# pyannote/pyannote-audio

Hardware: AMD Instinct MI355X
Metric: audio-hours/sec (real-time factor) for speaker-diarization-3.1 pipeline (higher is better)
Workload: dtype f32

## Files before the change

include/pyannote_amd.h:

```cpp
#ifndef PYANNOTE_AMD_H
#define PYANNOTE_AMD_H

#include <stddef.h>
#include <stdint.h>

#ifdef __cplusplus
extern "C" {
#endif

int pa_version(void);
const char* pa_last_error(void);

void pa_prof_enable(int on);
size_t pa_prof_report(char* buf, size_t cap);

#define PA_MAX_LSTM_LAYERS 8
#define PA_MAX_LINEAR 4

typedef struct pa_seg_weights {
  int32_t sinc_stride;
  int32_t lstm_layers;
  int32_t lstm_hidden;
  int32_t lstm_bidir;
  int32_t num_linear;
// ... 31 lines not shown
                 float* mean, float* rstd, void* stream);
int pa_sinc_fir_pool(const float* wav, long wav_len, long chunk_stride, int B, int N, int stride,
                     const float* mean, const float* rstd, float gamma, float beta,
                     const float* filt_packed, float* out, void* stream);
int pa_sinc_fir_span(const float* wav, long wav_len, long span, const float* filt_packed, float* S, void* stream);
int pa_sinc_fix_pool(const float* S, long Pc, int positions_per_chunk_step, int B, int P, const float* mean,
                     const float* rstd, float gamma, float beta, const float* filt_packed, float* tap_sums,
                     float* out, void* stream);
int pa_conv5_pool(const float* xin, int B, int cin, int Lin, const float* in_mean,
                  const float* in_rstd, const float* gam, const float* bet, const float* w_packed,
                  const float* bias64, float* out, void* stream);
int pa_norm_transpose(const float* xin, int B, int T, const float* in_mean, const float* in_rstd,
                      const float* gam, const float* bet, float* X0, void* stream);
int pa_gemm_tn_ex(const float* A, int lda, const float* W, int ldw, const float* bias, const float* Res,
                  float* C, long ldc, int M, int N, int K, int act, int out_mode, void* stream);
int pa_gemm_tn(const float* A, int lda, const float* W, int ldw, const float* bias, float* C, long ldc,
               int M, int N, int K, int act, int out_mode, void* stream);
int pa_gemm_tn_s2(const float* X, int B, int H, int W, int cin, const float* Wt, int ldw, const float* bias, float* C,
                  long ldc, int N, void* stream);
int pa_lstm_rec(const float* xproj, const float* whh_packed, float* out, int ntiles, int ndir, int T,
                void* stream);
int pa_lstm_rec_h(const float* xproj, const float* whh_packed, float* out, int ntiles, int ndir, int T, int H,
                  void* stream);
int pa_classifier(const float* X, int ldx, int K, int ntiles, int T, int B, const float* cw,
                  const float* cb, int NC, const unsigned char* mapping, int S, float* logp,
                  unsigned char* multilabel, void* stream);

#define PA_MAX_RES_BLOCKS 128

typedef struct pa_emb_weights {
  int32_t num_mel;
  int32_t embed_dim;
  int32_t num_layers;
  int32_t num_blocks[4];
  int32_t planes[4];
  int32_t bottleneck;
  const float* fb_window;
  const float* fb_tw256;
  const float* fb_tw512;
  const float* fb_mel_w;
  const int32_t* fb_mel_lo;
  const int32_t* fb_mel_hi;
  const float* stem_w;
  const float* stem_shift;
  const float* blk_w1[PA_MAX_RES_BLOCKS];
  const float* blk_shift1[PA_MAX_RES_BLOCKS];
  const float* blk_w2[PA_MAX_RES_BLOCKS];
  const float* blk_shift2[PA_MAX_RES_BLOCKS];
  const float* blk_u1[PA_MAX_RES_BLOCKS];
  const float* blk_u2[PA_MAX_RES_BLOCKS];
  const float* blk_wsc[PA_MAX_RES_BLOCKS];
  const float* blk_shiftsc[PA_MAX_RES_BLOCKS];
  const float* blk_w3[PA_MAX_RES_BLOCKS];
  const float* blk_shift3[PA_MAX_RES_BLOCKS];
  const float* seg1_w;
  const float* seg1_b;
  const float* blk_v1[PA_MAX_RES_BLOCKS];
  const float* blk_v2[PA_MAX_RES_BLOCKS];
  int32_t fb_center_kernel;
} pa_emb_weights;

int pa_emb_num_fbank_frames(int num_samples);
int pa_emb_num_pool_frames(const pa_emb_weights* w, int num_samples);
size_t pa_emb_workspace_bytes(const pa_emb_weights* w, int num_chunks, int num_samples, int num_masks);
int pa_emb_forward(const pa_emb_weights* w, const float* wav, int64_t wav_len, int64_t chunk_stride,
                   int num_chunks, int num_samples, const float* masks, int num_masks, int mask_frames,
                   const int32_t* nearest_idx, float* emb, void* workspace, size_t workspace_bytes,
                   void* stream);

size_t pa_emb_ragged_workspace_bytes(const pa_emb_weights* w, int num_utterances, int max_samples);
int pa_emb_forward_ragged(const pa_emb_weights* w, const float* wav, int64_t wav_len, const int64_t* offsets,
                          const int32_t* lengths, int num_utterances, int max_samples, const float* masks, float* emb,
                          void* workspace, size_t workspace_bytes, void* stream);

size_t pa_emb_calibrate_workspace_bytes(const pa_emb_weights* w, int num_chunks, int num_samples);
int pa_emb_calibrate_winograd(const pa_emb_weights* w, const float* wav, int64_t wav_len, int64_t chunk_stride,
                              int num_chunks, int num_samples, float* report, float* emb, void* workspace,
                              size_t workspace_bytes, void* stream);
int pa_absmax_diff(const float* got, const float* ref, long n, float* out2, void* stream);

int pa_fbank(const float* wav, long wav_len, long chunk_stride, int B, int N, const float* window,
             const float* tw256, const float* tw512, const float* mel_w, const int* mel_lo,
             const int* mel_hi, int nmel, float* out, int center, void* stream);
int pa_fbank_center_span(const float* fb, int B, int T, int nmel, int kernel, float* out, void* stream);
int pa_resnet_stem(const float* fbank, int B, int T, int F, const float* w9, const float* shift,
                   float* out, void* stream);
int pa_conv3x3(const float* X, int B, int H, int W, int cin, const float* Wg, const float* shift,
               const float* R, float* Y, int cout, int stride, int relu, void* stream);
int pa_winograd_pack_host(const float* conv_weight ,
                          const float* bn_scale , int cout, int cin,
                          float* U_slabs );
int pa_conv3x3_wino(const float* X, int B, int H, int W, int cin, const float* U, const float* shift,
                    const float* R, float* Y, int cout, int relu, void* stream);
int pa_winograd4_pack_host(const float* conv_weight ,
                           const float* bn_scale , int cout, int cin,
                           float* U_slabs );
int pa_conv3x3_wino4(const float* X, int B, int H, int W, int cin, const float* U, const float* shift,
                     const float* R, float* Y, int cout, int relu, void* stream);
int pa_conv3x3_wino4_rows(const float* X, int B, int H, int W, int cin, const float* U, const float* shift,
                          const float* R, float* Y, int cout, int relu, int rows, void* stream);
int pa_conv3x3_wino_rows(const float* X, int B, int H, int W, int cin, const float* U, const float* shift,
                         const float* R, float* Y, int cout, int relu, int y_first, void* stream);
int pa_stats_pool(const float* feat, int B, int Fh, int Tp, int C, const float* masks, int S, int Fm,
                  const int* nearest_idx, float* stats, void* stream);
int pa_fbank_ragged(const float* wav, long wav_len, const int64_t* offsets, const int32_t* lengths, int B,
                    int max_samples, const float* window, const float* tw256, const float* tw512, const float* mel_w,
                    const int* mel_lo, const int* mel_hi, int nmel, float* out, void* stream);
int pa_zero_tail_cols(float* x, int B, int H, int W, int C, const int32_t* lengths, int halvings, void* stream);
int pa_stats_pool_ragged(const float* feat, int B, int Fh, int W, int C, const int32_t* lengths, int halvings,
                         const float* masks, int ld_masks, float* stats, void* stream);

#define PA_W2V_MAX_CONV 8
#define PA_W2V_MAX_LAYERS 24
typedef struct pa_w2v_layer {
  const float* qk_w;
  const float* qk_b;
  const float* v_w;
  const float* out_w;
  const float* out_b;
  const float* ln1_g;
  const float* ln1_b;
  const float* ff1_w;
  const float* ff1_b;
  const float* ff2_w;
  const float* ff2_b;
  const float* ln2_g;
  const float* ln2_b;
  const float* gate_w;
  const float* gate_b;
  const float* gate_const;
} pa_w2v_layer;

typedef struct pa_sser_weights {
  int32_t num_conv;
  int32_t conv_channels[PA_W2V_MAX_CONV];
  int32_t conv_kernel[PA_W2V_MAX_CONV];
  int32_t conv_stride[PA_W2V_MAX_CONV];
  int32_t extractor_layer_norm;
  int32_t embed_dim, num_layers, num_heads, ff_dim, layer_norm_first;
  int32_t pos_kernel, pos_groups;
  int32_t wavlm;
  int32_t use_layer;
  int32_t lstm_layers, lstm_hidden, lstm_bidir, num_linear, linear_hidden, num_classes, num_speakers;
  const float* conv_w[PA_W2V_MAX_CONV];
  const float* conv_b[PA_W2V_MAX_CONV];
  const float* conv_norm_g[PA_W2V_MAX_CONV];
  const float* conv_norm_b[PA_W2V_MAX_CONV];
  const float* proj_ln_g;
  const float* proj_ln_b;
  const float* proj_w;
  const float* proj_b;
  const float* pos_w;
  const float* pos_b;
  const float* enc_ln_g;
  const float* enc_ln_b;
  pa_w2v_layer layers[PA_W2V_MAX_LAYERS];
  float layer_mix[PA_W2V_MAX_LAYERS];
  const float* lstm_wih[PA_MAX_LSTM_LAYERS];
  const float* lstm_bias[PA_MAX_LSTM_LAYERS];
  const float* lstm_whh[PA_MAX_LSTM_LAYERS];
  const float* lin_w[PA_MAX_LINEAR];
  const float* lin_b[PA_MAX_LINEAR];
  const float* cls_w;
  const float* cls_b;
  const uint8_t* powerset_map;
} pa_sser_weights;
// ... 138 lines not shown
```

pyannote-audio_amd/csrc/emb_fbank.hip:

```cpp
#include "common.h"

namespace pa {

constexpr int FB_WIN = 400, FB_SHIFT = 160, FB_NFFT = 512, FB_HALF = 256, FB_NBIN = 257;
constexpr int FB_FPB = 4;

struct cplx {
  float x, y;
};
__device__ __forceinline__ cplx cmul(cplx a, cplx b) {
  return {a.x * b.x - a.y * b.y, a.x * b.y + a.y * b.x};
}

template <bool kRagged>
__global__ __launch_bounds__(256) void k_fbank(const float* __restrict__ wav, long wav_len,
                                               long chunk_stride, int T, float scale, float preemph,
                                               const float* __restrict__ window,
                                               const float2* __restrict__ tw256,
                                               const float2* __restrict__ tw512,
                                               const float* __restrict__ mel_w,
                                               const int* __restrict__ mel_lo,
                                               const int* __restrict__ mel_hi, int nmel, float eps,
                                               float* __restrict__ out, const int64_t* __restrict__ offs,
                                               const int* __restrict__ lens) {
// ... 61 lines not shown
  }
  __syncthreads();

  float2* src = A;
  float2* dst = Bf;
#pragma unroll
  for (int pass = 0; pass < 4; ++pass) {
    const int Ns = 1 << (2 * pass);
    const int j = lane;
    const int k = j & (Ns - 1);
    const int tstep = 64 >> (2 * pass);
    cplx v[4];
#pragma unroll
    for (int r = 0; r < 4; ++r) {
      const float2 d = src[j + 64 * r];
      const float2 w = s_tw256[(r * k * tstep) & 255];
      v[r] = cmul({d.x, d.y}, {w.x, w.y});
    }
    const cplx t0 = {v[0].x + v[2].x, v[0].y + v[2].y};
    const cplx t1 = {v[0].x - v[2].x, v[0].y - v[2].y};
    const cplx t2 = {v[1].x + v[3].x, v[1].y + v[3].y};
    const cplx d13 = {v[1].x - v[3].x, v[1].y - v[3].y};
    const cplx t3 = {d13.y, -d13.x};
    const int j0 = ((j - k) << 2) + k;
    dst[j0] = make_float2(t0.x + t2.x, t0.y + t2.y);
    dst[j0 + Ns] = make_float2(t1.x + t3.x, t1.y + t3.y);
    dst[j0 + 2 * Ns] = make_float2(t0.x - t2.x, t0.y - t2.y);
    dst[j0 + 3 * Ns] = make_float2(t1.x - t3.x, t1.y - t3.y);
    __syncthreads();
    float2* tmp = src;
    src = dst;
    dst = tmp;
  }
#pragma unroll
  for (int i = 0; i < 5; ++i) {
    const int k = lane + 64 * i;
    if (k <= FB_HALF) {
      const float2 zk = src[k & 255];
      const float2 zc0 = src[(FB_HALF - k) & 255];
      const cplx zc = {zc0.x, -zc0.y};
      const cplx e = {0.5f * (zk.x + zc.x), 0.5f * (zk.y + zc.y)};
      const cplx dd = {0.5f * (zk.x - zc.x), 0.5f * (zk.y - zc.y)};
      const cplx o = {dd.y, -dd.x};
      const float2 w = w512[i];
      const cplx wo = cmul(o, {w.x, w.y});
      const float re = e.x + wo.x, im = e.y + wo.y;
      xw[k] = re * re + im * im;
    }
  }
  __syncthreads();
  if (active) {
    for (int m = lane; m < nmel; m += 64) {
      const float* wrow = mel_w + (long)m * FB_NBIN;
      float acc = 0.f;
      const int lo = mel_lo[m], hi = mel_hi[m];
      for (int k0 = lo; k0 <= hi; k0 += 8) {
        float wk[8];
#pragma unroll
        for (int u = 0; u < 8; ++u) wk[u] = k0 + u <= hi ? wrow[k0 + u] : 0.f;
#pragma unroll
        for (int u = 0; u < 8; ++u)
          if (k0 + u <= hi) acc = fmaf(xw[k0 + u], wk[u], acc);
      }
      out[((long)b * T + t) * nmel + m] = logf(fmaxf(acc, eps));
    }
  }
}

__global__ __launch_bounds__(320) void k_fbank_center(float* __restrict__ fb, int T, int nmel) {
  __shared__ float part[4][80];
  const int b = blockIdx.x;
  const int m = threadIdx.x % 80, p = threadIdx.x / 80;
  float* x = fb + (long)b * T * nmel;
  float s = 0.f;
  if (m < nmel)
    for (int t = p; t < T; t += 4) s += x[(long)t * nmel + m];
  part[p][m] = s;
  __syncthreads();
  const float mean = (part[0][m] + part[1][m] + part[2][m] + part[3][m]) / (float)T;
  if (m < nmel)
    for (int t = p; t < T; t += 4) x[(long)t * nmel + m] -= mean;
}

__global__ __launch_bounds__(320) void k_fbank_center_ragged(float* __restrict__ fb, int T, int nmel,
                                                             const int* __restrict__ lens) {
  __shared__ float part[4][80];
  const int b = blockIdx.x;
  const int m = threadIdx.x % 80, p = threadIdx.x / 80;
  const int n = lens[b];
  const int Tb = n < FB_WIN ? 0 : 1 + (n - FB_WIN) / FB_SHIFT;
  float* x = fb + (long)b * T * nmel;
  float s = 0.f;
  if (m < nmel)
    for (int t = p; t < Tb; t += 4) s += x[(long)t * nmel + m];
  part[p][m] = s;
  __syncthreads();
  const float mean = (part[0][m] + part[1][m] + part[2][m] + part[3][m]) / (float)Tb;
  if (m < nmel) {
    for (int t = p; t < Tb; t += 4) x[(long)t * nmel + m] -= mean;
    for (int t = Tb + p; t < T; t += 4) x[(long)t * nmel + m] = 0.f;
  }
}

constexpr int FC_TT = 240, FC_MG = 16, FC_KMAX = 2049;
__global__ __launch_bounds__(256) void k_fbank_center_span(const float* __restrict__ fb, int T, int nmel, int K,
                                                           float* __restrict__ out) {
  extern __shared__ float fc_tile[];
  const int b = blockIdx.z, m0 = blockIdx.y * FC_MG, t0 = blockIdx.x * FC_TT;
  const int half = K >> 1;
  const int m = threadIdx.x & (FC_MG - 1), tl = threadIdx.x >> 4;
  const float* x = fb + (long)b * T * nmel;
  const int rows = FC_TT + K - 1;
  for (int r = tl; r < rows; r += 16) {
    const int t = t0 - half + r;
    fc_tile[r * FC_MG + m] = (t >= 0 && t < T && m0 + m < nmel) ? x[(long)t * nmel + m0 + m] : 0.f;
  }
  __syncthreads();
  if (m0 + m >= nmel) return;
  for (int i = tl; i < FC_TT; i += 16) {
    const int t = t0 + i;
    if (t >= T) break;
    const int lo = t - half < 0 ? 0 : t - half, hi = t + half > T - 1 ? T - 1 : t + half;
    float s = 0.f;
    for (int u = lo; u <= hi; ++u) s += fc_tile[(u - t0 + half) * FC_MG + m];
    out[((long)b * T + t) * nmel + m0 + m] = fc_tile[(i + half) * FC_MG + m] - s / (float)(hi - lo + 1);
  }
}

}

extern "C" {

int pa_fbank_center_span(const float* fb, int B, int T, int nmel, int kernel, float* out, void* stream) {
  PA_REQUIRE(kernel >= 1 && (kernel & 1), "pa_fbank_center_span: the window must be an odd number of frames (got %d)",
             kernel);
  PA_REQUIRE(fb != out, "pa_fbank_center_span: works out of place");
  if (B <= 0 || T <= 0 || nmel <= 0) return 0;
  if (kernel > 2 * T - 1) kernel = 2 * T - 1;
  PA_REQUIRE(kernel <= pa::FC_KMAX,
             "pa_fbank_center_span: a running mean over %d frames of a %d-frame chunk needs more than the LDS holds "
             "(at most %d frames)", kernel, T, pa::FC_KMAX);
  const size_t lds = (size_t)(pa::FC_TT + kernel - 1) * pa::FC_MG * sizeof(float);
  static bool attr_set = false;
  if (!attr_set) {
    (void)hipFuncSetAttribute((const void*)pa::k_fbank_center_span, hipFuncAttributeMaxDynamicSharedMemorySize,
                              (int)((pa::FC_TT + pa::FC_KMAX - 1) * pa::FC_MG * sizeof(float)));
    attr_set = true;
  }
  hipLaunchKernelGGL(pa::k_fbank_center_span, dim3(pa::cdiv(T, pa::FC_TT), pa::cdiv(nmel, pa::FC_MG), B), dim3(256), lds,
                     (hipStream_t)stream, fb, T, nmel, kernel, out);
  PA_CHECK_LAUNCH("pa_fbank_center_span");
  return 0;
}

int pa_fbank(const float* wav, long wav_len, long chunk_stride, int B, int N, const float* window,
             const float* tw256, const float* tw512, const float* mel_w, const int* mel_lo,
             const int* mel_hi, int nmel, float* out, int center, void* stream) {
  PA_REQUIRE(nmel <= 80, "pa_fbank: at most 80 mel bins are built (got %d)", nmel);
  if (B <= 0) return 0;
  PA_REQUIRE(N >= pa::FB_WIN, "pa_fbank: %d samples is shorter than one 25 ms frame", N);
  const int T = 1 + (N - pa::FB_WIN) / pa::FB_SHIFT;
  hipStream_t st = (hipStream_t)stream;
  pa::ProfScope prof("k_fbank", stream, (double)B * T * (5.0 * 512 * 9 + 2.0 * 257 * 3 + 2.0 * 257 * 2),
                     4.0 * B * N + 4.0 * B * T * nmel * (center ? 3 : 1));
  hipLaunchKernelGGL(pa::k_fbank<false>, dim3(pa::cdiv(T, pa::FB_FPB), B), dim3(256), 0, st, wav, wav_len,
                     chunk_stride, T, 32768.0f, 0.97f, window, (const float2*)tw256,
                     (const float2*)tw512, mel_w, mel_lo, mel_hi, nmel, 1.1920928955078125e-07f, out,
                     (const int64_t*)nullptr, (const int*)nullptr);
  PA_CHECK_LAUNCH("pa_fbank");
  if (center) {
    hipLaunchKernelGGL(pa::k_fbank_center, dim3(B), dim3(320), 0, st, out, T, nmel);
    PA_CHECK_LAUNCH("pa_fbank_center");
  }
  return 0;
}

int pa_fbank_ragged(const float* wav, long wav_len, const int64_t* offsets, const int32_t* lengths, int B,
                    int max_samples, const float* window, const float* tw256, const float* tw512, const float* mel_w,
                    const int* mel_lo, const int* mel_hi, int nmel, float* out, void* stream) {
  PA_REQUIRE(nmel <= 80, "pa_fbank_ragged: at most 80 mel bins are built (got %d)", nmel);
  if (B <= 0) return 0;
  PA_REQUIRE(max_samples >= pa::FB_WIN, "pa_fbank_ragged: %d samples is shorter than one 25 ms frame", max_samples);
  const int T = 1 + (max_samples - pa::FB_WIN) / pa::FB_SHIFT;
  hipStream_t st = (hipStream_t)stream;
  pa::ProfScope prof("k_fbank_ragged", stream, (double)B * T * (5.0 * 512 * 9 + 2.0 * 257 * 3 + 2.0 * 257 * 2),
                     4.0 * B * max_samples + 12.0 * B * T * nmel);
  hipLaunchKernelGGL(pa::k_fbank<true>, dim3(pa::cdiv(T, pa::FB_FPB), B), dim3(256), 0, st, wav, wav_len, 0L, T,
                     32768.0f, 0.97f, window, (const float2*)tw256, (const float2*)tw512, mel_w, mel_lo, mel_hi, nmel,
                     1.1920928955078125e-07f, out, offsets, (const int*)lengths);
  PA_CHECK_LAUNCH("pa_fbank_ragged");
  hipLaunchKernelGGL(pa::k_fbank_center_ragged, dim3(B), dim3(320), 0, st, out, T, nmel, (const int*)lengths);
  PA_CHECK_LAUNCH("pa_fbank_center_ragged");
  return 0;
}

}
```

pyannote-audio_amd/csrc/emb_forward.cpp:

```cpp
#include <hip/hip_runtime.h>
#include <stdint.h>
#include <stdlib.h>

#include "../../include/pyannote_amd.h"

namespace pa {
void set_error(const char* fmt, ...);
}

namespace {

struct EmbPlan {
  int B, N, T, F, S;
  int Hs[5], Ws[5];
  size_t fbank, act[4], stats, total, act_elems;
  size_t t2_off, gather_off;
};
inline size_t align64(size_t n) { return (n + 63) & ~(size_t)63; }

inline bool prefer_wino4(int H, int W, int cin) {
  auto up = [](int a, int b) { return (long)((a + b - 1) / b) * b; };
  long p4 = up(H, 4) * up(W, 64);
  const long p4_lin = up(H, 4) * up(W, 4);
  if (p4_lin * 120 <= p4 * 100) p4 = p4_lin * 120 / 100;
// ... 35 lines not shown
  for (int i = 0; i < 3; ++i) p->act[i] = take(p->act_elems);
  p->t2_off = p->gather_off = 0;
  if (w->bottleneck) {
    size_t t1 = 0, t2 = 0, g = 0;
    int cin = w->planes[0];
    for (int l = 0; l < w->num_layers; ++l) {
      const size_t planes = w->planes[l];
      const size_t in_px = (size_t)B * p->Hs[l == 0 ? 1 : l] * p->Ws[l == 0 ? 1 : l];
      const size_t out_px = (size_t)B * p->Hs[l + 1] * p->Ws[l + 1];
      t1 = t1 > in_px * planes ? t1 : in_px * planes;
      t2 = t2 > out_px * planes ? t2 : out_px * planes;
      if (l > 0) g = g > out_px * cin ? g : out_px * cin;
      cin = 4 * (int)planes;
    }
    p->t2_off = align64(t1);
    p->gather_off = p->t2_off + align64(t2);
    p->act[3] = take(p->gather_off + align64(g));
  } else if (calib) {
    p->act[3] = take(p->act_elems);
  }
  const int L = w->num_layers;
  p->stats = take((size_t)B * p->S * 2 * w->planes[L - 1] * ex * p->Hs[L]);
  p->total = o;
  return true;
}

}

extern "C" {

int pa_emb_num_fbank_frames(int num_samples) {
  return num_samples < 400 ? 0 : 1 + (num_samples - 400) / 160;
}

int pa_emb_num_pool_frames(const pa_emb_weights* w, int num_samples) {
  EmbPlan p;
  if (!make_plan(w, 1, num_samples, 1, &p)) return 0;
  return p.Ws[w->num_layers];
}

size_t pa_emb_workspace_bytes(const pa_emb_weights* w, int num_chunks, int num_samples, int num_masks) {
  EmbPlan p;
  if (!make_plan(w, num_chunks, num_samples, num_masks, &p)) return 0;
  return p.total * sizeof(float);
}

}

extern "C" int pa_absmax_diff(const float* got, const float* ref, long n, float* out2, void* stream);


static int emb_forward_impl(const pa_emb_weights* w, const float* wav, int64_t wav_len, int64_t chunk_stride,
                            int num_chunks, int num_samples, const float* masks, int num_masks, int mask_frames,
                            const int32_t* nearest_idx, float* emb, void* workspace, size_t workspace_bytes,
                            void* stream, float* calib, const int64_t* offsets = nullptr,
                            const int32_t* lengths = nullptr) {
  if (num_chunks <= 0) return 0;
  const bool ragged = lengths != nullptr;
  EmbPlan p;
  if (w->num_layers != 4 || !make_plan(w, num_chunks, num_samples, masks ? num_masks : 1, &p, calib != nullptr)) {
    pa::set_error("pa_emb_forward: %d samples is too short (fbank needs >= 400) or bad layer count",
                  num_samples);
    return 3;
  }
  if (workspace_bytes < p.total * sizeof(float)) {
    pa::set_error("pa_emb_forward: workspace too small (%zu < %zu bytes)", workspace_bytes,
                  p.total * sizeof(float));
    return 3;
  }
  float* ws = (float*)workspace;
  const int B = p.B;
  int rc;
#define RUN(call)           \
  do {                      \
    rc = (call);            \
    if (rc != 0) return rc; \
  } while (0)

  const int span = w->fb_center_kernel;
  if (ragged && span != 0) {
    pa::set_error("pa_emb_forward_ragged: fbank_centering_span checkpoints run one launch sequence per length");
    return 3;
  }
  if (ragged)
    RUN(pa_fbank_ragged(wav, wav_len, offsets, lengths, B, p.N, w->fb_window, w->fb_tw256, w->fb_tw512, w->fb_mel_w,
                        w->fb_mel_lo, w->fb_mel_hi, w->num_mel, ws + p.fbank, stream));
  else
    RUN(pa_fbank(wav, wav_len, chunk_stride, B, p.N, w->fb_window, w->fb_tw256, w->fb_tw512, w->fb_mel_w,
                 w->fb_mel_lo, w->fb_mel_hi, w->num_mel, ws + p.fbank, span == 0 ? 1 : 0, stream));
  auto zero_tail = [&](float* X, int l, int C) -> int {
    return ragged ? pa_zero_tail_cols(X, B, p.Hs[l], p.Ws[l], C, lengths, l > 0 ? l - 1 : 0, stream) : 0;
  };
  float* cur = ws + p.act[0];
  float* f1 = ws + p.act[1];
  float* f2 = ws + p.act[2];
  const float* feats = ws + p.fbank;
  if (span != 0) {
    RUN(pa_fbank_center_span(ws + p.fbank, B, p.T, p.F, span, f1, stream));
    feats = f1;
  }
  RUN(pa_resnet_stem(feats, B, p.T, p.F, w->stem_w, w->stem_shift, cur, stream));
  if (!w->bottleneck) RUN(zero_tail(cur, 0, w->planes[0]));

  auto conv_s1 = [&](const float* X, int H, int W, int ci, const float* v, const float* u, const float* wd,
                     const float* shift, const float* R, float* Y, int co, int slot) -> int {
    if (calib != nullptr) {
      float* scratch = ws + p.act[3];
      float* rep = calib + 4 * slot;
      const long n = (long)B * H * W * co;
      int r = pa_conv3x3(X, B, H, W, ci, wd, shift, R, Y, co, 1, 1, stream);
      if (r == 0 && v != nullptr) {
        r = pa_conv3x3_wino4(X, B, H, W, ci, v, shift, R, scratch, co, 1, stream);
        if (r == 0) r = pa_absmax_diff(scratch, Y, n, rep, stream);
      }
      if (r == 0 && u != nullptr) {
        r = pa_conv3x3_wino(X, B, H, W, ci, u, shift, R, scratch, co, 1, stream);
        if (r == 0) r = pa_absmax_diff(scratch, Y, n, rep + 2, stream);
      }
      return r;
    }
    if (v != nullptr && u != nullptr && H % 4 == 2 && H > 4 && split_rows_wanted() && prefer_wino4(H - 2, W, ci)) {
      const int r = pa_conv3x3_wino4_rows(X, B, H, W, ci, v, shift, R, Y, co, 1, H - 2, stream);
      return r != 0 ? r : pa_conv3x3_wino_rows(X, B, H, W, ci, u, shift, R, Y, co, 1, H - 2, stream);
    }
    if (v != nullptr && prefer_wino4(H, W, ci)) return pa_conv3x3_wino4(X, B, H, W, ci, v, shift, R, Y, co, 1, stream);
    if (u != nullptr) return pa_conv3x3_wino(X, B, H, W, ci, u, shift, R, Y, co, 1, stream);
    return pa_conv3x3(X, B, H, W, ci, wd, shift, R, Y, co, 1, 1, stream);
  };

  int blk = 0;
  int cin = w->planes[0];
  if (w->bottleneck) {
    float* nxt = f1;
    float* sc = f2;
    float* tmp = ws + p.act[3];
    for (int l = 0; l < w->num_layers; ++l) {
      const int planes = w->planes[l], cout = 4 * planes;
      for (int i = 0; i < w->num_blocks[l]; ++i, ++blk) {
        if (blk >= PA_MAX_RES_BLOCKS) {
          pa::set_error("pa_emb_forward: more than %d residual blocks", PA_MAX_RES_BLOCKS);
          return 3;
        }
        const int stride = (i == 0 && l > 0) ? 2 : 1;
        const int H = stride == 2 ? p.Hs[l] : p.Hs[l + 1], W = stride == 2 ? p.Ws[l] : p.Ws[l + 1];
        const int Ho = p.Hs[l + 1], Wo = p.Ws[l + 1];
        float* t1 = tmp;
        float* t2 = tmp + p.t2_off;
        RUN(pa_gemm_tn_ex(cur, cin, w->blk_w1[blk], cin, w->blk_shift1[blk], nullptr, t1, planes, B * H * W,
                          planes, cin, 2, 0, stream));
        RUN(zero_tail(t1, stride == 2 ? l : l + 1, planes));
        if (stride == 1 && w->blk_u2[blk] != nullptr)
          RUN(pa_conv3x3_wino(t1, B, H, W, planes, w->blk_u2[blk], w->blk_shift2[blk], nullptr, t2, planes, 1,
                              stream));
        else
          RUN(pa_conv3x3(t1, B, H, W, planes, w->blk_w2[blk], w->blk_shift2[blk], nullptr, t2, planes, stride,
                         1, stream));
        const float* res = cur;
        if (w->blk_wsc[blk] != nullptr) {
          if (stride == 2)
            RUN(pa_gemm_tn_s2(cur, B, H, W, cin, w->blk_wsc[blk], cin, w->blk_shiftsc[blk], sc, cout, cout, stream));
          else
            RUN(pa_gemm_tn_ex(cur, cin, w->blk_wsc[blk], cin, w->blk_shiftsc[blk], nullptr, sc, cout,
                              B * Ho * Wo, cout, cin, 0, 0, stream));
          res = sc;
        } else if (stride != 1 || cin != cout) {
          pa::set_error("pa_emb_forward: block %d needs a shortcut conv but none was given", blk);
          return 3;
        }
        RUN(pa_gemm_tn_ex(t2, planes, w->blk_w3[blk], planes, w->blk_shift3[blk], res, nxt, cout, B * Ho * Wo,
// ... 111 lines not shown
```

pyannote-audio_amd/ffi.py:

```python
from __future__ import annotations

import ctypes as C
from pathlib import Path

import torch

_LIB = None
PA_MAX_LSTM_LAYERS = 8
PA_MAX_LINEAR = 4

c_fp = C.c_void_p


class SegWeights(C.Structure):
    _fields_ = [
        ("sinc_stride", C.c_int32), ("lstm_layers", C.c_int32), ("lstm_hidden", C.c_int32),
        ("lstm_bidir", C.c_int32), ("num_linear", C.c_int32), ("linear_hidden", C.c_int32),
        ("num_classes", C.c_int32), ("num_speakers", C.c_int32),
        ("wav_gamma", C.c_float), ("wav_beta", C.c_float),
        ("sinc_filt", c_fp), ("norm0", c_fp), ("conv1_w", c_fp), ("conv1_b", c_fp), ("norm1", c_fp),
        ("conv2_w", c_fp), ("conv2_b", c_fp), ("norm2", c_fp),
        ("lstm_wih", c_fp * PA_MAX_LSTM_LAYERS), ("lstm_bias", c_fp * PA_MAX_LSTM_LAYERS),
        ("lstm_whh", c_fp * PA_MAX_LSTM_LAYERS),
        ("lin_w", c_fp * PA_MAX_LINEAR), ("lin_b", c_fp * PA_MAX_LINEAR),
# ... 81 lines not shown
    ]


class LibraryNotBuilt(RuntimeError):
    pass


def lib_path() -> Path:
    import os
    if os.environ.get("PA_LIB"):
        return Path(os.environ["PA_LIB"])
    return Path(__file__).resolve().parent / "libpyannote_amd.so"


def load():
    global _LIB
    if _LIB is not None:
        return _LIB
    p = lib_path()
    if not p.exists():
        raise LibraryNotBuilt(
            f"{p} not found: run `python -c 'import __graft_entry__ as g; g.build()'` "
            "(hipcc --offload-arch=gfx950).  There is no CPU fallback.")
    lib = C.CDLL(str(p))
    lib.pa_last_error.restype = C.c_char_p
    lib.pa_version.restype = C.c_int
    lib.pa_seg_workspace_bytes.restype = C.c_size_t
    lib.pa_seg_workspace_bytes.argtypes = [C.POINTER(SegWeights), C.c_int, C.c_int]
    lib.pa_seg_workspace_bytes_strided.restype = C.c_size_t
    lib.pa_seg_workspace_bytes_strided.argtypes = [C.POINTER(SegWeights), C.c_int, C.c_int, C.c_int64]
    lib.pa_seg_num_frames.argtypes = [C.c_int, C.c_int]
    lib.pa_seg_forward.argtypes = [C.POINTER(SegWeights), c_fp, C.c_int64, C.c_int64, C.c_int, C.c_int,
                                   c_fp, c_fp, c_fp, C.c_size_t, c_fp]
    lib.pa_row_stats.argtypes = [c_fp, C.c_long, C.c_long, C.c_int, C.c_int, C.c_float, c_fp, c_fp, c_fp]
    lib.pa_sinc_fir_pool.argtypes = [c_fp, C.c_long, C.c_long, C.c_int, C.c_int, C.c_int, c_fp, c_fp,
                                     C.c_float, C.c_float, c_fp, c_fp, c_fp]
    lib.pa_sinc_fir_span.argtypes = [c_fp, C.c_long, C.c_long, c_fp, c_fp, c_fp]
    lib.pa_sinc_fix_pool.argtypes = [c_fp, C.c_long, C.c_int, C.c_int, C.c_int, c_fp, c_fp, C.c_float, C.c_float,
                                     c_fp, c_fp, c_fp, c_fp]
    lib.pa_conv5_pool.argtypes = [c_fp, C.c_int, C.c_int, C.c_int, c_fp, c_fp, c_fp, c_fp, c_fp, c_fp,
                                  c_fp, c_fp]
    lib.pa_norm_transpose.argtypes = [c_fp, C.c_int, C.c_int, c_fp, c_fp, c_fp, c_fp, c_fp, c_fp]
    lib.pa_gemm_tn_ex.argtypes = [c_fp, C.c_int, c_fp, C.c_int, c_fp, c_fp, c_fp, C.c_long, C.c_int, C.c_int,
                                  C.c_int, C.c_int, C.c_int, c_fp]
    lib.pa_gemm_tn.argtypes = [c_fp, C.c_int, c_fp, C.c_int, c_fp, c_fp, C.c_long, C.c_int, C.c_int,
                               C.c_int, C.c_int, C.c_int, c_fp]
    lib.pa_lstm_rec.argtypes = [c_fp, c_fp, c_fp, C.c_int, C.c_int, C.c_int, c_fp]
    lib.pa_classifier.argtypes = [c_fp, C.c_int, C.c_int, C.c_int, C.c_int, C.c_int, c_fp, c_fp,
                                  C.c_int, c_fp, C.c_int, c_fp, c_fp, c_fp]
    lib.pa_prof_enable.argtypes = [C.c_int]
    lib.pa_prof_enable.restype = None
    lib.pa_prof_report.argtypes = [C.c_char_p, C.c_size_t]
    lib.pa_prof_report.restype = C.c_size_t
    _declare_optional(lib)
    _LIB = lib
    return lib


_OPTIONAL: list[tuple] = [
    ("pa_emb_num_fbank_frames", [C.c_int], C.c_int),
    ("pa_emb_num_pool_frames", [C.POINTER(EmbWeights), C.c_int], C.c_int),
    ("pa_emb_workspace_bytes", [C.POINTER(EmbWeights), C.c_int, C.c_int, C.c_int], C.c_size_t),
    ("pa_emb_forward", [C.POINTER(EmbWeights), c_fp, C.c_int64, C.c_int64, C.c_int, C.c_int, c_fp,
                        C.c_int, C.c_int, c_fp, c_fp, c_fp, C.c_size_t, c_fp], C.c_int),
    ("pa_emb_ragged_workspace_bytes", [C.POINTER(EmbWeights), C.c_int, C.c_int], C.c_size_t),
    ("pa_emb_forward_ragged", [C.POINTER(EmbWeights), c_fp, C.c_int64, c_fp, c_fp, C.c_int, C.c_int, c_fp, c_fp,
                               c_fp, C.c_size_t, c_fp], C.c_int),
    ("pa_fbank_ragged", [c_fp, C.c_long, c_fp, c_fp, C.c_int, C.c_int, c_fp, c_fp, c_fp, c_fp, c_fp, c_fp, C.c_int,
                         c_fp, c_fp], C.c_int),
    ("pa_zero_tail_cols", [c_fp, C.c_int, C.c_int, C.c_int, C.c_int, c_fp, C.c_int, c_fp], C.c_int),
    ("pa_stats_pool_ragged", [c_fp, C.c_int, C.c_int, C.c_int, C.c_int, c_fp, C.c_int, c_fp, C.c_int, c_fp, c_fp],
     C.c_int),
    ("pa_emb_calibrate_workspace_bytes", [C.POINTER(EmbWeights), C.c_int, C.c_int], C.c_size_t),
    ("pa_emb_calibrate_winograd", [C.POINTER(EmbWeights), c_fp, C.c_int64, C.c_int64, C.c_int, C.c_int, c_fp, c_fp,
                                   c_fp, C.c_size_t, c_fp], C.c_int),
    ("pa_lstm_rec_h", [c_fp, c_fp, c_fp, C.c_int, C.c_int, C.c_int, C.c_int, c_fp], C.c_int),
    ("pa_absmax_diff", [c_fp, c_fp, C.c_long, c_fp, c_fp], C.c_int),
    ("pa_gemm_tn_s2", [c_fp, C.c_int, C.c_int, C.c_int, C.c_int, c_fp, C.c_int, c_fp, c_fp, C.c_long, C.c_int,
                       c_fp], C.c_int),
    ("pa_gemm_tn_batched", [c_fp, C.c_int, C.c_long, C.c_long, c_fp, C.c_int, C.c_long, C.c_long, c_fp, c_fp, C.c_long,
                            C.c_long, C.c_long, C.c_int, C.c_int, C.c_int, C.c_int, C.c_int, C.c_int, c_fp], C.c_int),
    ("pa_fbank", [c_fp, C.c_long, C.c_long, C.c_int, C.c_int, c_fp, c_fp, c_fp, c_fp, c_fp, c_fp,
                  C.c_int, c_fp, C.c_int, c_fp], C.c_int),
    ("pa_fbank_center_span", [c_fp, C.c_int, C.c_int, C.c_int, C.c_int, c_fp, c_fp], C.c_int),
    ("pa_resnet_stem", [c_fp, C.c_int, C.c_int, C.c_int, c_fp, c_fp, c_fp, c_fp], C.c_int),
    ("pa_conv3x3", [c_fp, C.c_int, C.c_int, C.c_int, C.c_int, c_fp, c_fp, c_fp, c_fp, C.c_int, C.c_int,
                    C.c_int, c_fp], C.c_int),
    ("pa_conv3x3_wino", [c_fp, C.c_int, C.c_int, C.c_int, C.c_int, c_fp, c_fp, c_fp, c_fp, C.c_int, C.c_int,
                         c_fp], C.c_int),
    ("pa_conv3x3_wino4", [c_fp, C.c_int, C.c_int, C.c_int, C.c_int, c_fp, c_fp, c_fp, c_fp, C.c_int, C.c_int,
                          c_fp], C.c_int),
    ("pa_conv3x3_wino4_rows", [c_fp, C.c_int, C.c_int, C.c_int, C.c_int, c_fp, c_fp, c_fp, c_fp, C.c_int, C.c_int,
                               C.c_int, c_fp], C.c_int),
    ("pa_conv3x3_wino_rows", [c_fp, C.c_int, C.c_int, C.c_int, C.c_int, c_fp, c_fp, c_fp, c_fp, C.c_int, C.c_int,
                              C.c_int, c_fp], C.c_int),
    ("pa_pdist_f64", [c_fp, C.c_int, C.c_int, c_fp, c_fp], C.c_int),
    ("pa_cdist_cosine_f64", [c_fp, C.c_int, c_fp, C.c_int, C.c_int, c_fp, c_fp, c_fp], C.c_int),
    ("pa_centroid_means", [c_fp, C.c_int, c_fp, c_fp, C.c_int, c_fp, c_fp], C.c_int),
    ("pa_linkage_workspace_bytes", [C.c_int], C.c_size_t),
    ("pa_linkage_centroid_f64", [c_fp, C.c_int, c_fp, c_fp, C.c_size_t, c_fp], C.c_int),
    ("pa_linkage_centroid_f64_ex", [c_fp, C.c_int, c_fp, c_fp, C.c_size_t, C.c_int, c_fp], C.c_int),
    ("pa_seg_chunk_stats", [c_fp, C.c_int, C.c_int, C.c_int, c_fp, c_fp, c_fp], C.c_int),
    ("pa_embedding_masks", [c_fp, C.c_int, C.c_int, C.c_int, c_fp, C.c_int, C.c_int, c_fp, c_fp], C.c_int),
    ("pa_speaker_count", [c_fp, C.c_int, C.c_int, C.c_int, c_fp, C.c_int, c_fp, c_fp, c_fp], C.c_int),
    ("pa_cluster_activations", [c_fp, C.c_int, C.c_int, C.c_int, c_fp, c_fp, C.c_int, C.c_int, c_fp, c_fp],
     C.c_int),
    ("pa_topk_binarize", [c_fp, c_fp, C.c_int, C.c_int, C.c_int, c_fp, c_fp, c_fp], C.c_int),
    ("pa_topk_binarize_f32", [c_fp, c_fp, C.c_int, C.c_int, C.c_int, c_fp, c_fp, c_fp], C.c_int),
    ("pa_binarize_hysteresis", [c_fp, C.c_int, C.c_int, C.c_int, C.c_float, C.c_float, C.c_int, c_fp, c_fp],
     C.c_int),
    ("pa_cluster_max", [c_fp, C.c_int, C.c_int, C.c_int, c_fp, C.c_int, c_fp, c_fp], C.c_int),
    ("pa_aggregate", [c_fp, C.c_int, C.c_int, C.c_int, c_fp, C.c_int, c_fp, c_fp, C.c_float, C.c_float, C.c_int,
                      c_fp, c_fp], C.c_int),
    ("pa_binarize_regions_workspace_bytes", [C.c_int, C.c_int, C.c_int], C.c_size_t),
    ("pa_binarize_regions", [c_fp, C.c_int, C.c_int, c_fp, c_fp, c_fp, c_fp, C.c_double, C.c_double, C.c_double,
                             C.c_int, c_fp, c_fp, c_fp, c_fp, C.c_size_t, c_fp], C.c_int),
    ("pa_resample_poly", [c_fp, C.c_long, c_fp, C.c_int, C.c_int, C.c_int, C.c_int, c_fp, C.c_long, c_fp],
     C.c_int),
    ("pa_plda_transform", [c_fp, C.c_int, C.c_int, C.c_int, C.c_int, c_fp, c_fp, c_fp, c_fp, c_fp, c_fp, c_fp],
     C.c_int),
    ("pa_vbx_workspace_bytes", [C.c_int, C.c_int, C.c_int], C.c_size_t),
    ("pa_vbx_iteration", [c_fp, c_fp, C.c_int, C.c_int, C.c_int, C.c_double, C.c_double, C.c_int, c_fp, c_fp,
                          c_fp, C.c_size_t, c_fp], C.c_int),
    ("pa_stats_pool", [c_fp, C.c_int, C.c_int, C.c_int, C.c_int, c_fp, C.c_int, C.c_int, c_fp, c_fp,
                       c_fp], C.c_int),
    ("pa_stats_pool_rows", [c_fp, C.c_int, C.c_int, C.c_int, C.c_int, C.c_int, c_fp, C.c_int, C.c_int, c_fp,
                            c_fp, C.c_int, c_fp, c_fp, c_fp], C.c_int),
    ("pa_sser_num_frames", [C.POINTER(SserWeights), C.c_int], C.c_int),
    ("pa_sser_workspace_bytes", [C.POINTER(SserWeights), C.c_int, C.c_int], C.c_size_t),
    ("pa_sser_forward", [C.POINTER(SserWeights), c_fp, C.c_int64, C.c_int64, C.c_int, C.c_int, c_fp, c_fp, c_fp,
                         c_fp, C.c_size_t, c_fp], C.c_int),
    ("pa_xvec_num_frames", [C.POINTER(XvecWeights), C.c_int], C.c_int),
    ("pa_xvec_workspace_bytes", [C.POINTER(XvecWeights), C.c_int, C.c_int, C.c_int], C.c_size_t),
    ("pa_xvec_forward", [C.POINTER(XvecWeights), c_fp, C.c_int64, C.c_int64, C.c_int, C.c_int, c_fp,
                         C.c_int, C.c_int, c_fp, c_fp, c_fp, C.c_size_t, c_fp], C.c_int),
    ("pa_xvec_mfcc_num_frames", [C.POINTER(XvecMfccWeights), C.c_int], C.c_int),
    ("pa_xvec_mfcc_workspace_bytes", [C.POINTER(XvecMfccWeights), C.c_int, C.c_int, C.c_int], C.c_size_t),
    ("pa_xvec_mfcc_forward", [C.POINTER(XvecMfccWeights), c_fp, C.c_int64, C.c_int64, C.c_int, C.c_int, c_fp,
                              C.c_int, C.c_int, c_fp, c_fp, c_fp, C.c_size_t, c_fp], C.c_int),
    ("pa_mfcc_features", [C.POINTER(XvecMfccWeights), c_fp, C.c_int64, C.c_int64, C.c_int, C.c_int, c_fp, c_fp,
                          C.c_size_t, c_fp], C.c_int),
]


def _declare_optional(lib):
    for name, argtypes, restype in _OPTIONAL:
        if hasattr(lib, name):
            fn = getattr(lib, name)
            fn.argtypes = argtypes
            if restype is not None:
                fn.restype = restype


def ptr(t: torch.Tensor | None):
    if t is None:
        return None
    if not t.is_cuda:
        raise RuntimeError("libpyannote_amd kernels need device tensors (got a CPU tensor)")
    if not t.is_contiguous():
        raise RuntimeError("libpyannote_amd kernels need contiguous tensors")
    return C.c_void_p(t.data_ptr())


def stream():
    return C.c_void_p(torch.cuda.current_stream().cuda_stream)

# ... 45 lines not shown
```

Before: 1.302.

## Compute fbank frames once over the overlapping span and share them across chunks

When chunks overlap with a stride that is a multiple of the 160-sample hop, fbank frames are computed once for the whole contiguous span instead of once per chunk. A new centering kernel then gathers each chunk's rows from the shared frame buffer, subtracts the per-chunk mean and writes them out of place. This removes the redundant FFT and mel work on overlapping windows. It costs an extra scratch buffer (reusing an activation slot) and one extra read/write pass during centering.

```diff
diff --git a/include/pyannote_amd.h b/include/pyannote_amd.h
--- a/include/pyannote_amd.h
+++ b/include/pyannote_amd.h
@@ -137,6 +137,9 @@
 int pa_fbank(const float* wav, long wav_len, long chunk_stride, int B, int N, const float* window,
              const float* tw256, const float* tw512, const float* mel_w, const int* mel_lo,
              const int* mel_hi, int nmel, float* out, int center, void* stream);
+int pa_fbank_shared(const float* wav, long wav_len, long chunk_stride, int B, int N, const float* window,
+                    const float* tw256, const float* tw512, const float* mel_w, const int* mel_lo,
+                    const int* mel_hi, int nmel, float* frames, float* out, void* stream);
 int pa_fbank_center_span(const float* fb, int B, int T, int nmel, int kernel, float* out, void* stream);
 int pa_resnet_stem(const float* fbank, int B, int T, int F, const float* w9, const float* shift,
                    float* out, void* stream);
diff --git a/pyannote-audio_amd/csrc/emb_fbank.hip b/pyannote-audio_amd/csrc/emb_fbank.hip
--- a/pyannote-audio_amd/csrc/emb_fbank.hip
+++ b/pyannote-audio_amd/csrc/emb_fbank.hip
@@ -167,6 +167,23 @@
     for (int t = p; t < T; t += 4) x[(long)t * nmel + m] -= mean;
 }
 
+__global__ __launch_bounds__(320) void k_fbank_center_rows(const float* __restrict__ frames, long rows_per_chunk,
+                                                           float* __restrict__ out, int T, int nmel) {
+  __shared__ float part[4][80];
+  const int b = blockIdx.x;
+  const int m = threadIdx.x % 80, p = threadIdx.x / 80;
+  const float* x = frames + (long)b * rows_per_chunk * nmel;
+  float* y = out + (long)b * T * nmel;
+  float s = 0.f;
+  if (m < nmel)
+    for (int t = p; t < T; t += 4) s += x[(long)t * nmel + m];
+  part[p][m] = s;
+  __syncthreads();
+  const float mean = (part[0][m] + part[1][m] + part[2][m] + part[3][m]) / (float)T;
+  if (m < nmel)
+    for (int t = p; t < T; t += 4) y[(long)t * nmel + m] = x[(long)t * nmel + m] - mean;
+}
+
 __global__ __launch_bounds__(320) void k_fbank_center_ragged(float* __restrict__ fb, int T, int nmel,
                                                              const int* __restrict__ lens) {
   __shared__ float part[4][80];
@@ -260,6 +277,32 @@
   return 0;
 }
 
+int pa_fbank_shared(const float* wav, long wav_len, long chunk_stride, int B, int N, const float* window,
+                    const float* tw256, const float* tw512, const float* mel_w, const int* mel_lo,
+                    const int* mel_hi, int nmel, float* frames, float* out, void* stream) {
+  PA_REQUIRE(nmel <= 80, "pa_fbank_shared: at most 80 mel bins are built (got %d)", nmel);
+  if (B <= 0) return 0;
+  PA_REQUIRE(N >= pa::FB_WIN, "pa_fbank_shared: %d samples is shorter than one 25 ms frame", N);
+  PA_REQUIRE(chunk_stride > 0 && chunk_stride % pa::FB_SHIFT == 0,
+             "pa_fbank_shared: the chunk stride (%ld) must be a positive multiple of the %d-sample hop", chunk_stride,
+             pa::FB_SHIFT);
+  PA_REQUIRE(frames != out, "pa_fbank_shared: works out of place");
+  const int T = 1 + (N - pa::FB_WIN) / pa::FB_SHIFT;
+  const long rows = chunk_stride / pa::FB_SHIFT;
+  const long G = (long)(B - 1) * rows + T;
+  PA_REQUIRE(G <= 0x7fffffffL - pa::FB_FPB, "pa_fbank_shared: %ld frames in one span", G);
+  hipStream_t st = (hipStream_t)stream;
+  pa::ProfScope prof("k_fbank", stream, (double)G * (5.0 * 512 * 9 + 2.0 * 257 * 3 + 2.0 * 257 * 2),
+                     4.0 * ((double)(G - 1) * pa::FB_SHIFT + pa::FB_WIN) + 4.0 * G * nmel + 8.0 * B * T * nmel);
+  hipLaunchKernelGGL(pa::k_fbank<false>, dim3(pa::cdiv(G, pa::FB_FPB), 1), dim3(256), 0, st, wav, wav_len, 0L, (int)G,
+                     32768.0f, 0.97f, window, (const float2*)tw256, (const float2*)tw512, mel_w, mel_lo, mel_hi, nmel,
+                     1.1920928955078125e-07f, frames, (const int64_t*)nullptr, (const int*)nullptr);
+  PA_CHECK_LAUNCH("pa_fbank_shared");
+  hipLaunchKernelGGL(pa::k_fbank_center_rows, dim3(B), dim3(320), 0, st, (const float*)frames, rows, out, T, nmel);
+  PA_CHECK_LAUNCH("pa_fbank_center_rows");
+  return 0;
+}
+
 int pa_fbank_ragged(const float* wav, long wav_len, const int64_t* offsets, const int32_t* lengths, int B,
                     int max_samples, const float* window, const float* tw256, const float* tw512, const float* mel_w,
                     const int* mel_lo, const int* mel_hi, int nmel, float* out, void* stream) {
diff --git a/pyannote-audio_amd/csrc/emb_forward.cpp b/pyannote-audio_amd/csrc/emb_forward.cpp
--- a/pyannote-audio_amd/csrc/emb_forward.cpp
+++ b/pyannote-audio_amd/csrc/emb_forward.cpp
@@ -141,9 +141,15 @@
     pa::set_error("pa_emb_forward_ragged: fbank_centering_span checkpoints run one launch sequence per length");
     return 3;
   }
+  const int64_t hop_rows = chunk_stride / 160;
+  const bool shared_frames = !ragged && span == 0 && B > 1 && chunk_stride > 0 && chunk_stride % 160 == 0 &&
+                             chunk_stride < num_samples && hop_rows <= p.T;
   if (ragged)
     RUN(pa_fbank_ragged(wav, wav_len, offsets, lengths, B, p.N, w->fb_window, w->fb_tw256, w->fb_tw512, w->fb_mel_w,
                         w->fb_mel_lo, w->fb_mel_hi, w->num_mel, ws + p.fbank, stream));
+  else if (shared_frames)
+    RUN(pa_fbank_shared(wav, wav_len, chunk_stride, B, p.N, w->fb_window, w->fb_tw256, w->fb_tw512, w->fb_mel_w,
+                        w->fb_mel_lo, w->fb_mel_hi, w->num_mel, ws + p.act[1], ws + p.fbank, stream));
   else
     RUN(pa_fbank(wav, wav_len, chunk_stride, B, p.N, w->fb_window, w->fb_tw256, w->fb_tw512, w->fb_mel_w,
                  w->fb_mel_lo, w->fb_mel_hi, w->num_mel, ws + p.fbank, span == 0 ? 1 : 0, stream));
diff --git a/pyannote-audio_amd/ffi.py b/pyannote-audio_amd/ffi.py
--- a/pyannote-audio_amd/ffi.py
+++ b/pyannote-audio_amd/ffi.py
@@ -187,6 +187,8 @@
                             C.c_long, C.c_long, C.c_int, C.c_int, C.c_int, C.c_int, C.c_int, C.c_int, c_fp], C.c_int),
     ("pa_fbank", [c_fp, C.c_long, C.c_long, C.c_int, C.c_int, c_fp, c_fp, c_fp, c_fp, c_fp, c_fp,
                   C.c_int, c_fp, C.c_int, c_fp], C.c_int),
+    ("pa_fbank_shared", [c_fp, C.c_long, C.c_long, C.c_int, C.c_int, c_fp, c_fp, c_fp, c_fp, c_fp, c_fp,
+                         C.c_int, c_fp, c_fp, c_fp], C.c_int),
     ("pa_fbank_center_span", [c_fp, C.c_int, C.c_int, C.c_int, C.c_int, c_fp, c_fp], C.c_int),
     ("pa_resnet_stem", [c_fp, C.c_int, C.c_int, C.c_int, c_fp, c_fp, c_fp, c_fp], C.c_int),
     ("pa_conv3x3", [c_fp, C.c_int, C.c_int, C.c_int, C.c_int, c_fp, c_fp, c_fp, c_fp, C.c_int, C.c_int,
```

Result: no change. 1.311 (median of 6 runs) (+0.7%).
